# Dunni3/FlowMol

Hardware: AMD Instinct MI355X
Metric: molecules/sec at 250 timesteps (GEOM-drugs-sized graphs) (higher is better)
Workload: dtype f32

## Files before the change

flowmol_amd/csrc/fm_kernels.h:

```cpp
#pragma once
#include <type_traits>

#include "../../include/flowmol_hip.h"
#include "fm_device.h"

struct FmBatch {
    int B, N, E, U;
    int P;
    int n_tiles, tile_rows;
    const int* mol_node_off;
    const int* mol_edge_off;
    const int* mol_pair_off;
    int* node_mol;
    int* node_first_edge;
    int* e_src;
    int* e_dst;
    int* e_pair;
    int* p_e0;
    int* p_e1;
    int* pair_mol;
    const int* mol_tile_off;
    int4* tile_desc;
};

#define FM_CHUNK_E 16

static __global__ void __launch_bounds__(256) fm_k_batch_setup(FmBatch b) {
    const int gid = blockIdx.x * blockDim.x + threadIdx.x;
    if (gid < b.N) {
        int lo = 0, hi = b.B;
        while (hi - lo > 1) { const int mid = (lo + hi) >> 1; if (b.mol_node_off[mid] <= gid) lo = mid; else hi = mid; }
        b.node_mol[gid] = lo;
        const int n = b.mol_node_off[lo + 1] - b.mol_node_off[lo];
        b.node_first_edge[gid] = b.mol_edge_off[lo] + (gid - b.mol_node_off[lo]) * (n - 1);
    }
    if (gid < b.E) {
        int lo = 0, hi = b.B;
        while (hi - lo > 1) { const int mid = (lo + hi) >> 1; if (b.mol_edge_off[mid] <= gid) lo = mid; else hi = mid; }
        const int noff = b.mol_node_off[lo];
        const int n = b.mol_node_off[lo + 1] - noff;
        const int local = gid - b.mol_edge_off[lo];
        const int i = local / (n - 1), k = local % (n - 1);
        const int j = k + (k >= i ? 1 : 0);
        b.e_dst[gid] = noff + i;
        b.e_src[gid] = noff + j;
        const int a = i < j ? i : j, c = i < j ? j : i;
        const int pair = b.mol_pair_off[lo] + a * (2 * n - a - 1) / 2 + (c - a - 1);
        b.e_pair[gid] = pair;
        if (j < i) { b.p_e0[pair] = gid; b.pair_mol[pair] = lo; }
        else b.p_e1[pair] = gid;
    }
    if (gid < b.n_tiles) {
        int lo = 0, hi = b.B;
        while (hi - lo > 1) { const int mid = (lo + hi) >> 1; if (b.mol_tile_off[mid] <= gid) lo = mid; else hi = mid; }
        const int moff = b.mol_edge_off[lo];
        const int e0 = moff + (gid - b.mol_tile_off[lo]) * b.tile_rows;
        const int left = b.mol_edge_off[lo + 1] - e0;
        b.tile_desc[gid] = make_int4(e0, left < b.tile_rows ? left : b.tile_rows, moff, lo);
    }
}

enum FmMlpMode {
    FM_MLP_TABLE = 0,
    FM_MLP_SC_NODE = 1,
    FM_MLP_NODE_HEAD = 2,
    FM_MLP_EDGE_HEAD = 3,
    FM_MLP_SC_EDGE = 4,
    FM_MLP_NODE_LOSS = 5,
    FM_MLP_EDGE_LOSS = 6,
};
constexpr bool fm_mlp_node_head(int mode) { return mode == FM_MLP_NODE_HEAD || mode == FM_MLP_NODE_LOSS; }
constexpr bool fm_mlp_edge_head(int mode) { return mode == FM_MLP_EDGE_HEAD || mode == FM_MLP_EDGE_LOSS; }

__device__ __forceinline__ int fm_loss_target(const int* tok_t, const int* tok_1, int row, int mask) { return tok_t[row] == mask ? tok_1[row] : -1; }
template <bool LOSS>
__device__ __forceinline__ void fm_head_row(const float* lg, int n, float* out, int target) {
    if (LOSS && target < 0) { out[0] = 0.f; return; }
    float m = lg[0];
    for (int c = 1; c < n; ++c) m = fmaxf(m, lg[c]);
    float s = 0.f;
    for (int c = 0; c < n; ++c) s += expf(lg[c] - m);
    if (LOSS) out[0] = (logf(s) + m) - lg[target];
    else for (int c = 0; c < n; ++c) out[c] = expf(lg[c] - m) / s;
}

struct FmMlpArgs {
    int rows;
    int K1p;
    int H;
    int O;
    int ldx, ldh;
    const float2* W1; const float* b1;
    const float2* W2; const float* b2;
    const float* ln_g; const float* ln_b; int ln_n;
    const float* in;  int in_ld;
    int in_w;
    float* out; int out_ld;
    const float* s_tab; const int* tok_a; const int* tok_c; int n_c1;
    const float* prev_a; const float* prev_c; const float* prev_x; const float* x_t;
    int na, nc, ne;
    float rbf_mu_step, rbf_inv_sigma;
    float* out2;
    const float* ef; const int* p_e0; const int* p_e1;
    const int* e_src; const int* e_dst; const int* e_pair; const int* tok_e;
    const float* prev_e; const float* T1; const float* ef_tab;
    const float* emb_a; const float* emb_c; const float* temb; int ta, tc, tt;
    const float2* slabW0; float* slabQ0; const float2* slabW1; float* slabQ1;
    int tab_tiles; int tab_stride;
    const int* tab_slot; const int* node_mol; int slot_rows;
    const int* tgt_a; const int* tgt_c; const int* tgt_e;
};

template <int MODE, int TM>
__device__ __forceinline__ void fm_mlp2_tile(const FmMlpArgs& a, int tile, float* lds) {
    float* X = lds;
    float* Hb = lds + TM * a.ldx;
    int* meta = reinterpret_cast<int*>(Hb + TM * a.ldh);
    const int tid = threadIdx.x;
    const int row0 = tile * TM;

    if (MODE == FM_MLP_TABLE) {
        for (int idx = tid; idx < TM * a.K1p; idx += FM_THREADS) {
            const int r = idx / a.K1p, c = idx % a.K1p, row = row0 + r;
            float v = 0.f;
            if (row < a.rows) {
                if (a.in) v = (a.in_w == 0 || c < a.in_w) ? a.in[(size_t)row * a.in_ld + c] : 0.f;
                else {
                    const int ia = row / a.n_c1, ic = row % a.n_c1;
                    if (c < a.ta) v = a.emb_a ? a.emb_a[ia * a.ta + c] : (c == ia ? 1.f : 0.f);
                    else if (c < a.ta + a.tc) v = a.emb_c ? a.emb_c[ic * a.tc + (c - a.ta)] : ((c - a.ta) == ic ? 1.f : 0.f);
                    else if (c < a.ta + a.tc + a.tt) v = a.temb[c - a.ta - a.tc];
                }
            }
            X[r * a.ldx + c] = v;
        }
    } else if (MODE == FM_MLP_SC_NODE) {
        float* dd = reinterpret_cast<float*>(meta + TM);
        if (tid < TM) {
            const int n = row0 + tid;
            int tok = -1; float d = 0.f;
            if (n < a.rows) {
                tok = a.tok_a[n] * a.n_c1 + a.tok_c[n];
                if (a.tab_slot) tok += a.tab_slot[a.node_mol[n]] * a.slot_rows;
                d = fm_norm3(a.x_t[n * 3 + 0] - a.prev_x[n * 3 + 0], a.x_t[n * 3 + 1] - a.prev_x[n * 3 + 1], a.x_t[n * 3 + 2] - a.prev_x[n * 3 + 2]);
            }
            meta[tid] = tok; dd[tid] = d;
        }
        __syncthreads();
        {
            const auto rs = fm_buf(a.s_tab, 0x7fffffffu);
            constexpr int NQ = TM * 64 / FM_THREADS;
            float4 q[NQ];
#pragma unroll
            for (int k = 0; k < NQ; ++k) {
                const int idx = tid + k * FM_THREADS, r = idx >> 6, c4 = idx & 63;
                const int tok = meta[r];
                q[k] = fm_buf_f32x4(rs, tok >= 0 ? tok * 1024 + c4 * 16 : FM_BUF_OOB, 0);
            }
#pragma unroll
            for (int k = 0; k < NQ; ++k) {
                const int idx = tid + k * FM_THREADS, r = idx >> 6, c4 = idx & 63;
                *reinterpret_cast<float4*>(X + r * a.ldx + c4 * 4) = q[k];
            }
        }
        const int kin = a.na + a.nc + 32, kw = a.K1p - 256;
        for (int idx = tid; idx < TM * kw; idx += FM_THREADS) {
            const int r = idx / kw, c = idx % kw;
            const int n = row0 + r;
            float v = 0.f;
            if (meta[r] >= 0 && c < kin) {
                if (c < a.na) v = a.prev_a[(size_t)n * a.na + c];
                else if (c < a.na + a.nc) v = a.prev_c[(size_t)n * a.nc + (c - a.na)];
                else v = fm_rbf(dd[r], c - a.na - a.nc, a.rbf_mu_step, a.rbf_inv_sigma);
            }
            X[r * a.ldx + 256 + c] = v;
        }
    } else if (fm_mlp_node_head(MODE)) {
        const int left = a.rows - row0;
        const auto rs = fm_buf(a.in + (size_t)row0 * 256, (unsigned)(left < TM ? left : TM) * 1024u);
        constexpr int NQ = TM * 64 / FM_THREADS;
        float4 q[NQ];
#pragma unroll
        for (int k = 0; k < NQ; ++k) q[k] = fm_buf_f32x4(rs, (tid + k * FM_THREADS) * 16, 0);
#pragma unroll
        for (int k = 0; k < NQ; ++k) {
            const int idx = tid + k * FM_THREADS, r = idx >> 6, c4 = idx & 63;
            *reinterpret_cast<float4*>(X + r * a.ldx + c4 * 4) = q[k];
        }
    } else if (fm_mlp_edge_head(MODE)) {
        int* pr = meta + 3 * TM;
        if (tid < TM) {
            const int p = row0 + tid;
            meta[tid] = (p < a.rows) ? a.p_e0[p] : -1;
            pr[tid] = (p < a.rows) ? a.p_e1[p] : -1;
        }
        __syncthreads();
        constexpr int NQ = TM * 32 / FM_THREADS;
        float4 u0[NQ], u1[NQ];
#pragma unroll
        for (int k = 0; k < NQ; ++k) {
            const int idx = tid + k * FM_THREADS, r = idx >> 5, c4 = idx & 31;
            const int ea = meta[r], eb = pr[r];
            u0[k] = reinterpret_cast<const float4*>(a.ef)[(size_t)(ea < 0 ? 0 : ea) * 32 + c4];
            u1[k] = reinterpret_cast<const float4*>(a.ef)[(size_t)(eb < 0 ? 0 : eb) * 32 + c4];
        }
#pragma unroll
        for (int k = 0; k < NQ; ++k) {
            const int idx = tid + k * FM_THREADS, r = idx >> 5, c4 = idx & 31;
            const bool ok = meta[r] >= 0;
            float4 v;
            v.x = ok ? u0[k].x + u1[k].x : 0.f; v.y = ok ? u0[k].y + u1[k].y : 0.f;
            v.z = ok ? u0[k].z + u1[k].z : 0.f; v.w = ok ? u0[k].w + u1[k].w : 0.f;
            *reinterpret_cast<float4*>(X + r * a.ldx + 4 * c4) = v;
        }
    } else {
        float* dd = reinterpret_cast<float*>(meta + TM);
        int* pr = meta + 3 * TM;
        if (tid < TM) {
            const int p = row0 + tid;
            int tok = -1, ea = -1, eb = -1;
            float dt_ = 0.f, d1_ = 0.f;
            if (p < a.rows) {
                ea = a.p_e0[p]; eb = a.p_e1[p];
                const int i = a.e_src[ea], j = a.e_dst[ea];
                tok = a.tok_e[p];
                dt_ = fm_norm3(a.x_t[i * 3] - a.x_t[j * 3], a.x_t[i * 3 + 1] - a.x_t[j * 3 + 1], a.x_t[i * 3 + 2] - a.x_t[j * 3 + 2]) + 1e-8f;
                d1_ = fm_norm3(a.prev_x[i * 3] - a.prev_x[j * 3], a.prev_x[i * 3 + 1] - a.prev_x[j * 3 + 1],
                               a.prev_x[i * 3 + 2] - a.prev_x[j * 3 + 2]) + 1e-8f;
            }
            meta[tid] = tok; pr[tid] = eb; dd[2 * tid] = dt_; dd[2 * tid + 1] = d1_;
            meta[4 * TM + tid] = ea;
        }
        __syncthreads();
        for (int idx = tid; idx < TM * a.K1p; idx += FM_THREADS) {
            const int r = idx / a.K1p, c = idx % a.K1p;
            float v = 0.f;
            if (meta[r] >= 0) {
                if (c < a.ne) v = a.prev_e[(size_t)(row0 + r) * a.ne + c];
                else if (c < a.ne + 32)
                    v = fm_rbf(dd[2 * r + 1], c - a.ne, a.rbf_mu_step, a.rbf_inv_sigma) -
                        fm_rbf(dd[2 * r], c - a.ne, a.rbf_mu_step, a.rbf_inv_sigma);
            }
            X[r * a.ldx + c] = v;
        }
    }
    __syncthreads();

    fm_block_gemm<TM / 16, 1>(X, a.ldx, TM / 16, a.K1p / 8, a.W1, a.H / 16, [&](int row, int col, float v) {
        if (MODE == FM_MLP_SC_EDGE) { const int t = meta[row]; v += (t >= 0) ? a.T1[t * 128 + col] : 0.f; }
        else v += a.b1[col];
        Hb[row * a.ldh + col] = fm_silu(v);
    });
    __syncthreads();
    auto epi2 = [&](int row, int col, float v) {
        v += a.b2[col];
        if (MODE == FM_MLP_TABLE || MODE == FM_MLP_SC_NODE || MODE == FM_MLP_SC_EDGE) v = fm_silu(v);
        X[row * a.ldx + col] = v;
    };
    if (fm_mlp_node_head(MODE) || fm_mlp_edge_head(MODE)) fm_block_gemm<1, 1>(Hb, a.ldh, TM / 16, a.H / 8, a.W2, a.O / 16, epi2);
    else fm_block_gemm<TM / 16, 1>(Hb, a.ldh, TM / 16, a.H / 8, a.W2, a.O / 16, epi2);
    __syncthreads();

    constexpr int LPR = FM_THREADS / TM;
    const int r = tid / LPR, sub = tid % LPR;
    const int grow = row0 + r;
    if (MODE == FM_MLP_TABLE) {
        float mean, rstd;
        fm_row_stats<LPR>(X + r * a.ldx, a.ln_n, sub, mean, rstd);
        if (grow < a.rows) {
            float* o0 = a.out + (size_t)(a.p_e0 ? a.p_e0[grow] : grow) * a.out_ld;
            float* o1 = a.p_e1 ? a.out + (size_t)a.p_e1[grow] * a.out_ld : nullptr;
            for (int c = sub; c < a.O; c += LPR) {
                const float y = fm_fma((X[r * a.ldx + c] - mean) * rstd, a.ln_g[c], a.ln_b[c]);
                o0[c] = y;
                if (o1) o1[c] = y;
            }
        }
    } else if (MODE == FM_MLP_SC_NODE) {
        if (grow < a.rows) {
            const float* trow = a.s_tab + (size_t)meta[r] * 256;
            for (int c = sub * 4; c < 256; c += LPR * 4) {
                const float4 t = *reinterpret_cast<const float4*>(trow + c);
                const float4 x = *reinterpret_cast<const float4*>(X + r * a.ldx + c);
                *reinterpret_cast<float4*>(a.out + (size_t)grow * 256 + c) = make_float4(t.x + x.x, t.y + x.y, t.z + x.z, t.w + x.w);
            }
        }
    } else if (MODE == FM_MLP_SC_EDGE) {
        const bool slab = a.slabQ0 != nullptr;
        if (grow < a.rows) {
            const int ea = meta[4 * TM + r], eb = meta[3 * TM + r], tok = meta[r];
            for (int c = sub * 4; c < 128; c += LPR * 4) {
                const float4 t = *reinterpret_cast<const float4*>(a.ef_tab + tok * 128 + c);
                const float4 x = *reinterpret_cast<const float4*>(X + r * a.ldx + c);
                const float4 o = make_float4(t.x + x.x, t.y + x.y, t.z + x.z, t.w + x.w);
                *reinterpret_cast<float4*>(a.out + (size_t)ea * 128 + c) = o;
                *reinterpret_cast<float4*>(a.out + (size_t)eb * 128 + c) = o;
                if (slab) *reinterpret_cast<float4*>(Hb + r * a.ldh + 32 + c) = o;
            }
        }
        if (slab) {
            const float* dd = reinterpret_cast<const float*>(meta + TM);
            for (int idx = tid; idx < TM * 32; idx += FM_THREADS) {
                const int rr = idx >> 5, k = idx & 31;
                Hb[rr * a.ldh + k] = fm_rbf(dd[2 * rr], k, a.rbf_mu_step, a.rbf_inv_sigma);
            }
            __syncthreads();
            const int lane = tid & 63, wave = __builtin_amdgcn_readfirstlane(tid >> 6);
            const int left = a.rows - row0;
            auto slab_gemm = [&](const float2* __restrict__ W, float* Q) {
                constexpr int MT = TM / 16;
                f32x4 acc[MT][2];
#pragma unroll
                for (int i = 0; i < MT; ++i) { acc[i][0] = f32x4{0.f, 0.f, 0.f, 0.f}; acc[i][1] = f32x4{0.f, 0.f, 0.f, 0.f}; }
                fm_wave_gemm<MT, 2>(acc, Hb, 164, 20, W, 16, 2 * wave, lane);
                const auto rs = fm_buf(Q + (size_t)row0 * 256, (unsigned)(left < TM ? left : TM) * 1024u);
#pragma unroll
                for (int i = 0; i < MT; ++i)
#pragma unroll
                    for (int q = 0; q < 4; ++q)
                        fm_buf_store_f32x2(rs, (i * 16 + 4 * (lane >> 4) + q) * 1024 + (lane & 15) * 8, wave * 128, acc[i][0][q], acc[i][1][q]);
            };
            slab_gemm(a.slabW0, a.slabQ0);
            if (a.slabQ1) slab_gemm(a.slabW1, a.slabQ1);
        }
    } else {
        if (sub == 0 && grow < a.rows) {
            const float* lg = X + r * a.ldx;
            if (MODE == FM_MLP_NODE_HEAD) {
                fm_head_row<false>(lg, a.na, a.out + (size_t)grow * a.na, 0);
                fm_head_row<false>(lg + a.na, a.nc, a.out2 + (size_t)grow * a.nc, 0);
            } else if (MODE == FM_MLP_EDGE_HEAD) {
                fm_head_row<false>(lg, a.ne, a.out + (size_t)grow * a.ne, 0);
            } else if (MODE == FM_MLP_NODE_LOSS) {
                fm_head_row<true>(lg, a.na, a.out + grow, fm_loss_target(a.tok_a, a.tgt_a, grow, a.na));
                fm_head_row<true>(lg + a.na, a.nc, a.out2 + grow, fm_loss_target(a.tok_c, a.tgt_c, grow, a.nc));
            } else {
                fm_head_row<true>(lg, a.ne, a.out + grow, fm_loss_target(a.tok_e, a.tgt_e, grow, a.ne));
            }
        }
    }
}

template <int MODE, int TM = FM_TM>
__global__ void __launch_bounds__(FM_THREADS) fm_k_mlp2(FmMlpArgs a) {
    HIP_DYNAMIC_SHARED(float, lds)
    int tile = blockIdx.x;
    if (MODE == FM_MLP_TABLE && a.tab_tiles > 0) {
        const int tab = tile / a.tab_tiles;
        tile -= tab * a.tab_tiles;
        a.temb += tab * a.tt;
        a.out += (size_t)tab * a.tab_stride;
    }
    fm_mlp2_tile<MODE, TM>(a, tile, lds);
}

template <int MODE_A, int MODE_B, int TM = FM_TM>
__global__ void __launch_bounds__(FM_THREADS) fm_k_mlp2_pair(FmMlpArgs a, FmMlpArgs b, int tiles_a) {
    HIP_DYNAMIC_SHARED(float, lds)
    if ((int)blockIdx.x < tiles_a) fm_mlp2_tile<MODE_A, TM>(a, blockIdx.x, lds);
    else fm_mlp2_tile<MODE_B, TM>(b, (int)blockIdx.x - tiles_a, lds);
}

enum FmMlp4Mode { FM_MLP4_SC_NODE = 0, FM_MLP4_NODE_HEAD = 1, FM_MLP4_PROJ0 = 2, FM_MLP4_NODE_LOSS = 3 };
struct FmMlp4Args {
    int N;
    const void* W1q; const float* b1;
    const void* W2q; const float* b2;
    const float* s_tab; const int* tok_a; const int* tok_c; int n_c1;
    const int* tab_slot; const int* node_mol; int slot_rows;
    const float* prev_a; const float* prev_c; const float* prev_x; const float* x_t;
    int na, nc; float rbf_mu_step, rbf_inv_sigma;
    float* out; float* out2;
    const float* in;
    const void* Wps4; float* Ps; float* PV; int pv_w; float* v_init; int V; const float* x_src; float* x_dst;
    const int* tgt_a; const int* tgt_c;
};
#define FM_MLP4_LDX 324
#define FM_MLP4_LDH 260
#define FM_MLP4_LDS_BYTES ((4 * FM_MLP4_LDX + 4 * FM_MLP4_LDH + 16) * 4)

template <int MODE>
__device__ __forceinline__ void fm_mlp4_tile(const FmMlp4Args& a, int tile, float* lds) {
    constexpr int LDX = FM_MLP4_LDX, LDH = FM_MLP4_LDH;
    float* X = lds;
    float* Hb = X + 4 * LDX;
    int* meta = reinterpret_cast<int*>(Hb + 4 * LDH);
    float* dd = reinterpret_cast<float*>(meta + 4);
    const int tid = threadIdx.x, row0 = tile * 4;
    const int rows = a.N - row0 < 4 ? a.N - row0 : 4;
    if (MODE == FM_MLP4_SC_NODE) {
        if (tid < 4) {
            const int n = row0 + tid;
            int tok = -1; float d = 0.f;
            if (n < a.N) {
                tok = a.tok_a[n] * a.n_c1 + a.tok_c[n];
                if (a.tab_slot) tok += a.tab_slot[a.node_mol[n]] * a.slot_rows;
                d = fm_norm3(a.x_t[n * 3 + 0] - a.prev_x[n * 3 + 0], a.x_t[n * 3 + 1] - a.prev_x[n * 3 + 1], a.x_t[n * 3 + 2] - a.prev_x[n * 3 + 2]);
            }
            meta[tid] = tok; dd[tid] = d;
        }
        __syncthreads();
        if (tid < 256) {
            const int r = tid >> 6, c4 = tid & 63, tok = meta[r];
            *reinterpret_cast<float4*>(X + r * LDX + c4 * 4) = fm_buf_f32x4(fm_buf(a.s_tab), tok >= 0 ? tok * 1024 + c4 * 16 : FM_BUF_OOB, 0);
        } else {
            const int r = (tid - 256) >> 6, c = (tid - 256) & 63, n = row0 + r;
            float v = 0.f;
            if (meta[r] >= 0 && c < a.na + a.nc + 32) {
                if (c < a.na) v = a.prev_a[(size_t)n * a.na + c];
                else if (c < a.na + a.nc) v = a.prev_c[(size_t)n * a.nc + (c - a.na)];
                else v = fm_rbf(dd[r], c - a.na - a.nc, a.rbf_mu_step, a.rbf_inv_sigma);
            }
            X[r * LDX + 256 + c] = v;
        }
    } else {
        if (tid < 256)
            *reinterpret_cast<float4*>(X + (tid >> 6) * LDX + (tid & 63) * 4) = fm_buf_f32x4(fm_buf(a.in + (size_t)row0 * 256, (unsigned)rows * 1024u), tid * 16, 0);
        if (MODE == FM_MLP4_PROJ0) {
            for (int i = tid; i < rows * 3; i += FM_THREADS) a.x_dst[row0 * 3 + i] = a.x_src[row0 * 3 + i];
            for (int i = tid; i < rows * 3 * a.V; i += FM_THREADS) a.v_init[(size_t)row0 * 3 * a.V + i] = 0.f;
            for (int i = tid; i < rows * 3 * a.pv_w; i += FM_THREADS) a.PV[(size_t)row0 * 3 * a.pv_w + i] = 0.f;
        }
    }
    __syncthreads();
    if (MODE == FM_MLP4_PROJ0) {
        fm_rows4_linear<64, 4>(X, LDX, a.Wps4, [&](int r, int c, float v) { if (r < rows) a.Ps[(size_t)(row0 + r) * 256 + c] = v; });
        return;
    }
    if (MODE == FM_MLP4_SC_NODE)
        fm_rows4_linear<80, 4>(X, LDX, a.W1q, [&](int r, int c, float v) { Hb[r * LDH + c] = fm_silu(v + a.b1[c]); });
    else
        fm_rows4_linear<64, 4>(X, LDX, a.W1q, [&](int r, int c, float v) { Hb[r * LDH + c] = fm_silu(v + a.b1[c]); });
    if (MODE == FM_MLP4_SC_NODE) {
        fm_rows4_linear<64, 4>(Hb, LDH, a.W2q, [&](int r, int c, float v) {
            if (r < rows) a.out[(size_t)(row0 + r) * 256 + c] = a.s_tab[(size_t)meta[r] * 256 + c] + fm_silu(v + a.b2[c]);
        });
    } else {
        const int no = a.na + a.nc;
        fm_rows4_linear<64, 1>(Hb, LDH, a.W2q, [&](int r, int c, float v) { if (c < no) X[r * LDX + c] = v + a.b2[c]; });
        if (tid < rows) {
            const float* lg = X + tid * LDX;
            const int n = row0 + tid;
            if (MODE == FM_MLP4_NODE_LOSS) {
                fm_head_row<true>(lg, a.na, a.out + n, fm_loss_target(a.tok_a, a.tgt_a, n, a.na));
                fm_head_row<true>(lg + a.na, a.nc, a.out2 + n, fm_loss_target(a.tok_c, a.tgt_c, n, a.nc));
            } else {
                fm_head_row<false>(lg, a.na, a.out + (size_t)n * a.na, 0);
                fm_head_row<false>(lg + a.na, a.nc, a.out2 + (size_t)n * a.nc, 0);
            }
        }
    }
}

template <int MODE>
__global__ void __launch_bounds__(FM_THREADS) fm_k_mlp4(FmMlp4Args a) {
    HIP_DYNAMIC_SHARED(float, lds)
    fm_mlp4_tile<MODE>(a, blockIdx.x, lds);
}

template <int MODE4, int MODE_B>
__global__ void __launch_bounds__(FM_THREADS) fm_k_mlp4_pair(FmMlp4Args a, FmMlpArgs b, int tiles_a) {
    HIP_DYNAMIC_SHARED(float, lds)
    if ((int)blockIdx.x < tiles_a) fm_mlp4_tile<MODE4>(a, blockIdx.x, lds);
    else fm_mlp2_tile<MODE_B, 16>(b, (int)blockIdx.x - tiles_a, lds);
}

static __global__ void __launch_bounds__(256) fm_k_gather_rows(float* __restrict__ out, const float* __restrict__ tab, int width,
                                                         int rows, const int* __restrict__ tok_a, const int* __restrict__ tok_c,
                                                         int n_c1, const int* __restrict__ e_pair, const int* __restrict__ tab_slot,
                                                         const int* __restrict__ node_mol, int slot_rows) {
    const int w4 = width / 4;
    for (size_t idx = (size_t)blockIdx.x * blockDim.x + threadIdx.x; idx < (size_t)rows * w4; idx += (size_t)gridDim.x * blockDim.x) {
        const int row = (int)(idx / w4), c4 = (int)(idx % w4);
        int tok = e_pair ? tok_a[e_pair[row]] : tok_a[row] * n_c1 + tok_c[row];
        if (tab_slot) tok += tab_slot[node_mol[row]] * slot_rows;
        reinterpret_cast<float4*>(out)[idx] = reinterpret_cast<const float4*>(tab)[(size_t)tok * w4 + c4];
    }
}

struct FmProjArgs {
    int N;
    const float* s; const float* v;
    const float2* Wps; float* Ps;
    const float2* Wasd; float* Asd;
    const float2* Wpv; float* PV;
    int pv_w;
    float* v_init;
    const float* x_src; float* x_dst;
};

template <int V, int TM = FM_TM>
__global__ void __launch_bounds__(FM_THREADS) fm_k_node_proj(FmProjArgs a) {
    HIP_DYNAMIC_SHARED(float, lds)
    constexpr int LDS_ = 260;
    constexpr int LDV = V + 4;
    float* X = lds;
    float* Vt = lds + TM * LDS_;
    const int tid = threadIdx.x, row0 = blockIdx.x * TM;
    for (int idx = tid; idx < TM * 64; idx += FM_THREADS) {
        const int r = idx >> 6, c4 = idx & 63;
        float4 val = make_float4(0.f, 0.f, 0.f, 0.f);
        if (row0 + r < a.N) val = reinterpret_cast<const float4*>(a.s)[(size_t)(row0 + r) * 64 + c4];
        float* d = X + r * LDS_ + 4 * c4;
        *reinterpret_cast<float4*>(d) = val;
    }
    if (a.x_dst) {
        const int i0 = row0 * 3, i1 = (row0 + TM < a.N ? row0 + TM : a.N) * 3;
        for (int i = i0 + tid; i < i1; i += FM_THREADS) a.x_dst[i] = a.x_src[i];
    }
    if (a.PV) {
        const int rows = a.N - row0 < TM ? a.N - row0 : TM;
        const auto rs_v = fm_buf(a.v + (size_t)row0 * 3 * V, (unsigned)rows * (3 * V * 4));
        constexpr int V4 = V / 4, NCHK = TM * 3 * V4, NV = (NCHK + FM_THREADS - 1) / FM_THREADS;
        float4 qv[NV];
#pragma unroll
        for (int k = 0; k < NV; ++k) {
            const int idx = tid + k * FM_THREADS;
            if (a.v_init) {
                qv[k] = make_float4(0.f, 0.f, 0.f, 0.f);
                if (idx < rows * 3 * V4) reinterpret_cast<float4*>(a.v_init + (size_t)row0 * 3 * V)[idx] = qv[k];
            } else {
                qv[k] = fm_buf_f32x4(rs_v, idx < NCHK ? idx * 16 : FM_BUF_OOB, 0);
            }
        }
#pragma unroll
        for (int k = 0; k < NV; ++k) {
            const int idx = tid + k * FM_THREADS;
            if (idx < NCHK) {
                const int r = idx / (3 * V4), rem = idx % (3 * V4), c = rem / V4, u4 = rem % V4;
                *reinterpret_cast<float4*>(Vt + (c * TM + r) * LDV + u4 * 4) = qv[k];
            }
        }
    }
    __syncthreads();
    if (a.Ps)
        fm_block_gemm<TM / 16, 2>(X, LDS_, TM / 16, 32, a.Wps, 16, [&](int row, int col, float v) {
            if (row0 + row < a.N) a.Ps[(size_t)(row0 + row) * 256 + col] = v;
        });
    if (a.Asd)
        fm_block_gemm<TM / 16, 2>(X, LDS_, TM / 16, 32, a.Wasd, 16, [&](int row, int col, float v) {
            if (row0 + row < a.N) a.Asd[(size_t)(row0 + row) * 256 + col] = v;
        });
    if (a.PV)
        fm_block_gemm<1, 1>(Vt, LDV, 3 * TM / 16, V / 8, a.Wpv, a.pv_w / 16, [&](int row, int col, float v) {
            const int c = row / TM, r = row % TM;
            if (row0 + r < a.N) a.PV[((size_t)(row0 + r) * 3 + c) * a.pv_w + col] = v;
        });
}

struct FmDstProjArgs {
    int N;
    const float* s; const float* v;
    FmGvpW g;
    const float2* Wsd; float* Psd;
    const float2* Wpvd; float* PVd; int pv_w;
};

template <int V, int TM, int VD>
__global__ void __launch_bounds__(FM_THREADS) fm_k_dst_proj(FmDstProjArgs a) {
    typedef FmGvpTile<V, TM> T;
    HIP_DYNAMIC_SHARED(float, lds)
    float* X = lds;
    float* Vin = X + T::X_FLOATS;
    float* Vh = Vin + T::VIN_FLOATS;
    float* G = Vh + T::VH_FLOATS;
    const int tid = threadIdx.x, row0 = blockIdx.x * TM;
    {
        const int rows = a.N - row0 < TM ? a.N - row0 : TM;
        const auto rs_s = fm_buf(a.s + (size_t)row0 * 256, (unsigned)rows * 1024u);
        const auto rs_v = fm_buf(a.v + (size_t)row0 * 3 * V, (unsigned)rows * (3 * V * 4));
        constexpr int V4 = V / 4, NCHK = TM * 3 * V4;
        for (int idx = tid; idx < TM * 64; idx += FM_THREADS)
            *reinterpret_cast<float4*>(X + (idx >> 6) * FM_LDX + (idx & 63) * 4) = fm_buf_f32x4(rs_s, idx * 16, 0);
        for (int idx = tid; idx < NCHK; idx += FM_THREADS) {
            const int r = idx / (3 * V4), rem = idx % (3 * V4), c = rem / V4, u4 = rem % V4;
            *reinterpret_cast<float4*>(Vin + (c * TM + r) * T::LDVI + u4 * 4) = fm_buf_f32x4(rs_v, idx * 16, 0);
        }
    }
    __syncthreads();
    {
        FM_MARK_DECL
        float pre[TM / 16][2][4];
        fm_gvp_core<V, VD, false, true, TM, FM_THREADS>(X, Vin, Vh, G, a.g, pre FM_MARK_PASS(50));
    }
    constexpr int MT = TM / 16;
    fm_block_gemm<MT, 2>(X, FM_LDX, MT, 32, a.Wsd, 16, [&](int row, int col, float val) {
        if (row0 + row < a.N) a.Psd[(size_t)(row0 + row) * 256 + col] = val;
    });
    fm_block_gemm<1, 1>(Vin, T::LDVI, 3 * MT, 1, a.Wpvd, a.pv_w / 16, [&](int row, int col, float val) {
        const int c = row / TM, r = row % TM;
        if (row0 + r < a.N) a.PVd[((size_t)(row0 + r) * 3 + c) * a.pv_w + col] = val;
    });
}

struct FmMsgArgs {
    FmBatch b;
    const float* x;
    const float* ef;
    const float* Ps;
    const float* PV;
    const float* w0;
    const float* Psd;
    const float* PVd;
    FmGvpW g0, g1, g2;
    float* part_s;
    float* part_v;
    float rbf_mu_step, rbf_inv_sigma;
    float* dbg_s; float* dbg_v;
    const float* Q;
    int xcd_chunk;
};

template <int V, int TM, int NTH, int HX, int SP, int PQ = 0>
__global__ void __launch_bounds__(NTH) fm_k_edge_message(FmMsgArgs a) {
    static_assert(!(PQ && (SP || HX)), "the pair-slab instance exists for f32 models without destination features");
    typedef FmGvpTile<V, TM, HX> T;
    HIP_DYNAMIC_SHARED(float, lds)
    float* X = lds;
    constexpr int FMT = SP == 3 ? 1 : 0, NPL = SP == 2 ? 3 : 2;
    float* Vin = X + (SP ? TM * FM_LDP * NPL / 2 : T::X_FLOATS);
    float* Vh = Vin + T::VIN_FLOATS;
    float* G = SP ? Vh + TM * FM_LDG : Vh + T::VH_FLOATS;
    int* m_src = reinterpret_cast<int*>(SP ? Vh + T::VH_FLOATS : G + T::G_FLOATS);
    int* m_dst = m_src + TM;
    float* m_geo = reinterpret_cast<float*>(m_dst + TM);
    int* m_piece = reinterpret_cast<int*>(m_geo + 4 * TM);
    int* m_soff = m_piece + TM;
    int* m_doff = m_soff + TM;
    const int tid = threadIdx.x;
    const int tile = a.xcd_chunk > 0 ? (int)(blockIdx.x & 7) * a.xcd_chunk + (int)(blockIdx.x >> 3) : (int)blockIdx.x;
    if (tile >= a.b.n_tiles) return;
    const int4 td = a.b.tile_desc[tile];
    const int e0 = td.x, left = td.y, moff = td.z;
    FM_MARK_DECL
    constexpr int NEF = PQ ? 1 : TM * 32 / NTH;
    float4 efv[NEF];
    if constexpr (!PQ) {
        const auto rs = fm_buf(a.ef + (size_t)e0 * 128, (unsigned)left * 512u);
#pragma unroll
        for (int k = 0; k < NEF; ++k) efv[k] = (FM_ABLATE & 16) ? make_float4(0.1f, 0.2f, 0.3f, 0.4f) : fm_buf_f32x4(rs, tid * 16 + k * NTH * 16, 0);
    }
    if (PQ && tid < 64) {
        const int e = e0 + tid;
        const int pr = tid < left ? a.b.e_pair[e] : 0x7fffffff;
        int mn = pr;
#pragma unroll
        for (int o = 1; o < 64; o <<= 1) { const int t = __shfl_xor(mn, o); mn = t < mn ? t : mn; }
        if (tid < TM) m_doff[tid] = pr != 0x7fffffff ? (pr - mn) * 1024 : FM_BUF_OOB;
        if (tid == 0) m_doff[TM] = mn;
    }
    if (tid < TM) {
        const int e = e0 + tid;
        int s = -1, d = -1, piece = 0;
        float gx = 0.f, gy = 0.f, gz = 0.f, dist = 0.f;
        if (tid < left) {
            s = a.b.e_src[e]; d = a.b.e_dst[e];
            piece = (e - moff) / FM_CHUNK_E - (a.b.node_first_edge[d] - moff) / FM_CHUNK_E;
            const float dx = a.x[s * 3] - a.x[d * 3], dy = a.x[s * 3 + 1] - a.x[d * 3 + 1], dz = a.x[s * 3 + 2] - a.x[d * 3 + 2];
            dist = fm_norm3(dx, dy, dz) + 1e-8f;
            const float inv_d = __builtin_amdgcn_rcpf(dist);
            gx = dx * inv_d; gy = dy * inv_d; gz = dz * inv_d;
        }
        m_src[tid] = s; m_dst[tid] = d; m_piece[tid] = piece;
        m_soff[tid] = s >= 0 ? s * 1024 : FM_BUF_OOB;
        if (!PQ) m_doff[tid] = d >= 0 ? d * 1024 : FM_BUF_OOB;
        m_geo[4 * tid] = gx; m_geo[4 * tid + 1] = gy; m_geo[4 * tid + 2] = gz; m_geo[4 * tid + 3] = dist;
    }
    __syncthreads();
    FM_MARK(0);
    float pre[TM / 16][1024 / NTH][4];
    if (!(FM_ABLATE & 16)) fm_gather_pre<TM, NTH, false>(pre, a.Ps, a.b.N, m_soff);
    else { for (auto& p1 : pre) for (auto& p2 : p1) for (auto& p3 : p2) p3 = 0.25f; }
    if (HX > 0) fm_gather_pre<TM, NTH, true>(pre, a.Psd, a.b.N, m_doff);
    float preq[PQ ? TM / 16 : 1][PQ ? 1024 / NTH : 1][4];
    if constexpr (PQ) {
        static_assert(!PQ || NTH == 512, "Q rows are laid out for 8 waves x 2 column tiles");
        const int pmin = __builtin_amdgcn_readfirstlane(m_doff[TM]);
        const int lane = tid & 63, wave = __builtin_amdgcn_readfirstlane(tid >> 6);
        const auto rs = fm_buf(a.Q + (size_t)pmin * 256, 0x7ffffc00u);
#pragma unroll
        for (int i = 0; i < TM / 16; ++i)
#pragma unroll
            for (int r = 0; r < 4; ++r) {
                const float2 t = fm_buf_f32x2(rs, m_doff[i * 16 + 4 * (lane >> 4) + r] + (lane & 15) * 8, wave * 128);
                preq[i][0][r] = t.x; preq[i][1][r] = t.y;
            }
    }
    {
        constexpr int PVW = T::PVW, CB = PVW / 16, NCH = 3 * CB * TM, QN = NTH / 16, NP = (NCH + QN - 1) / QN;
        const int q = tid >> 4, j = tid & 15;
        const auto rs = fm_buf(a.PV, (unsigned)a.b.N * (unsigned)(3 * PVW * 4));
        const auto rsd = fm_buf(HX > 0 ? a.PVd : a.PV, (unsigned)a.b.N * (unsigned)(3 * PVW * 4));
        float pv[NP], w0v[NP];
#pragma unroll
        for (int p_ = 0; p_ < NP; ++p_) {
            const int ch = q + p_ * QN, r = ch % TM, ccb = ch / TM, c = ccb / CB, cb = ccb % CB;
            const int sidx = (NCH % QN == 0 || ch < NCH) ? m_src[r] : -1;
            pv[p_] = (FM_ABLATE & 16) ? 0.5f : fm_buf_f32(rs, sidx >= 0 ? sidx * (3 * PVW * 4) + j * 4 : FM_BUF_OOB, (c * PVW + cb * 16) * 4);
            if (HX > 0) {
                const int didx = (NCH % QN == 0 || ch < NCH) ? m_dst[r] : -1;
                pv[p_] += fm_buf_f32(rsd, didx >= 0 ? didx * (3 * PVW * 4) + j * 4 : FM_BUF_OOB, (c * PVW + cb * 16) * 4);
            }
            w0v[p_] = a.w0[cb * 16 + j];
        }
#pragma unroll
        for (int p_ = 0; p_ < NP; ++p_) {
            const int ch = q + p_ * QN, r = ch % TM, ccb = ch / TM, c = ccb / CB, cb = ccb % CB;
            if (NCH % QN == 0 || ch < NCH)
                Vh[(c * TM + r) * T::LDVH + cb * 16 + j] = fm_fma(m_geo[4 * r + c], w0v[p_], pv[p_]);
        }
    }
    if (SP) {
        unsigned short* XH = reinterpret_cast<unsigned short*>(X);
        unsigned short* XL = XH + TM * FM_LDP;
        constexpr int Z0 = 160 + T::KU0, Z1 = 256 + T::KU;
        for (int idx = tid; idx < TM * 24; idx += NTH) {
            const int r = idx / 24, c = idx % 24;
            if (Z0 + c < (Z0 + 31) / 32 * 32) { XH[r * FM_LDP + Z0 + c] = 0; XL[r * FM_LDP + Z0 + c] = 0; if (SP == 2) XL[TM * FM_LDP + r * FM_LDP + Z0 + c] = 0; }
            if (Z1 + c < 320) { XH[r * FM_LDP + Z1 + c] = 0; XL[r * FM_LDP + Z1 + c] = 0; if (SP == 2) XL[TM * FM_LDP + r * FM_LDP + Z1 + c] = 0; }
        }
        for (int idx = tid; idx < TM * 32; idx += NTH) {
            const int r = idx >> 5, k = idx & 31;
            if (SP == 2) fm_split3_store(XH, XL, r, k, fm_rbf(m_geo[4 * r + 3], k, a.rbf_mu_step, a.rbf_inv_sigma));
            else fm_split_store<FM_LDP, FMT>(XH, XL, r, k, fm_rbf(m_geo[4 * r + 3], k, a.rbf_mu_step, a.rbf_inv_sigma));
        }
#pragma unroll
        for (int k = 0; k < NEF; ++k) {
            const int idx = tid + k * NTH, r = idx >> 5, c4 = idx & 31;
            if (SP == 2) {
                fm_split3_store(XH, XL, r, 32 + 4 * c4 + 0, efv[k].x); fm_split3_store(XH, XL, r, 32 + 4 * c4 + 1, efv[k].y);
                fm_split3_store(XH, XL, r, 32 + 4 * c4 + 2, efv[k].z); fm_split3_store(XH, XL, r, 32 + 4 * c4 + 3, efv[k].w);
            } else {
                fm_split_store<FM_LDP, FMT>(XH, XL, r, 32 + 4 * c4 + 0, efv[k].x); fm_split_store<FM_LDP, FMT>(XH, XL, r, 32 + 4 * c4 + 1, efv[k].y);
                fm_split_store<FM_LDP, FMT>(XH, XL, r, 32 + 4 * c4 + 2, efv[k].z); fm_split_store<FM_LDP, FMT>(XH, XL, r, 32 + 4 * c4 + 3, efv[k].w);
            }
        }
    } else if constexpr (!PQ) {
    for (int idx = tid; idx < TM * 32; idx += NTH) {
        const int r = idx >> 5, k = idx & 31;
        X[r * FM_LDX + k] = fm_rbf(m_geo[4 * r + 3], k, a.rbf_mu_step, a.rbf_inv_sigma);
    }
#pragma unroll
    for (int k = 0; k < NEF; ++k) {
        const int idx = tid + k * NTH, r = idx >> 5, c4 = idx & 31;
        *reinterpret_cast<float4*>(X + r * FM_LDX + 32 + 4 * c4) = efv[k];
    }
    }
    if constexpr (PQ) {
#pragma unroll
        for (int i = 0; i < TM / 16; ++i)
#pragma unroll
            for (int j = 0; j < 1024 / NTH; ++j)
#pragma unroll
                for (int r = 0; r < 4; ++r) pre[i][j][r] += preq[i][j][r];
    }
    __syncthreads();
    FM_MARK(1);
    constexpr bool PF = V == 32 && TM == 32 && NTH == 512 && SP == 0 && HX == 0;
    float2 bw[V / 8][2];
    fm_gvp_core_pf<V, V, true, true, TM, NTH, HX, SP, false, PQ != 0, 0, PF>(X, Vin, Vh, G, a.g0, a.g1, bw, pre FM_MARK_PASS(10));
    fm_gvp_core_pf<V, V, false, true, TM, NTH, HX, SP, false, false, 0, PF>(X, Vin, Vh, G, a.g1, a.g2, bw, pre FM_MARK_PASS(20));
    fm_gvp_core_pf<V, V, false, true, TM, NTH, HX, SP, true, false, 0, PF>(X, Vin, Vh, G, a.g2, a.g2, bw, pre FM_MARK_PASS(30));

    if (a.dbg_s) {
        for (int idx = tid; idx < TM * 256; idx += NTH) {
            const int r = idx >> 8, c = idx & 255;
            if (m_src[r] >= 0) a.dbg_s[(size_t)(e0 + r) * 256 + c] = X[r * FM_LDX + c];
        }
        for (int idx = tid; idx < 3 * TM * V; idx += NTH) {
            const int row = idx / V, u = idx % V, c = row / TM, r = row % TM;
            if (m_src[r] >= 0) a.dbg_v[((size_t)(e0 + r) * 3 + c) * V + u] = Vin[row * T::LDVI + u];
        }
    }
    FM_MARK(40);
    static_assert(NTH >= 512 && 3 * V <= 128 && TM <= 64, "waves 0..3 own the 256 scalar columns, waves 4..5 the 3*V vector columns (the others idle here; 1024-thread instances were measured in round 6: profiles/r06d_*)");
    if (!(FM_ABLATE & 8)) {
        const int wave = __builtin_amdgcn_readfirstlane(tid >> 6), lane = tid & 63;
        const int lr = lane < TM ? lane : TM - 1;
        const int myd = m_dst[lr];
        const int nxd = m_dst[lr + 1 < TM ? lr + 1 : TM - 1];
        const unsigned long long ends = __ballot(lane < TM && myd >= 0 && (lr + 1 == TM || nxd != myd || (lr & (FM_CHUNK_E - 1)) == FM_CHUNK_E - 1));
        const bool is_s = wave < 4;
        const int cv = tid - 256;
        auto column_sums = [&](const float* vp, auto stride_c, float* out_base, unsigned row_bytes, int col) {
            constexpr int STRIDE = decltype(stride_c)::value;
            float val[TM];
#pragma unroll
            for (int r = 0; r < TM; ++r) val[r] = vp[r * STRIDE];
            float run = 0.f;
#pragma unroll
            for (int r = 0; r < TM; ++r) {
                run += val[r];
                if ((ends >> r) & 1ull) {
                    const int d = __builtin_amdgcn_readfirstlane(m_dst[r]), pcr = __builtin_amdgcn_readfirstlane(m_piece[r]);
                    const size_t slot = (size_t)d * a.b.P + pcr;
                    fm_buf_store_f32(fm_buf(reinterpret_cast<const char*>(out_base) + slot * row_bytes, row_bytes), col * 4, 0, run);
                    run = 0.f;
                }
            }
        };
        if (is_s) column_sums(X + tid, std::integral_constant<int, FM_LDX>{}, a.part_s, 1024u, tid);
        else if (cv < 3 * V) column_sums(Vin + (cv / V) * TM * T::LDVI + (cv % V), std::integral_constant<int, T::LDVI>{}, a.part_v, 3 * V * 4u, cv);
    }
    FM_MARK(41);
}

struct FmNodeUpdArgs {
    FmBatch b;
    float* s; float* v;
    const float* part_s; const float* part_v;
    float inv_z;
    FmGvpW g0, g1, g2;
    const float* ln1_g; const float* ln1_b; const float* ln2_g; const float* ln2_b;
    float* agg_s; float* agg_v;
    const float2* Wps; float* Ps;
    const float2* Wpv; float* PV;
    const float2* Wasd; float* Asd;
    FmGvpW p0, p1, p2; float* x;
    const void* Wps_sp; const void* Wasd_sp;
    const void* Wps4; const void* Wasd4;
    int s_real;
};

template <int V, int TM, int SP = 0>
__device__ __forceinline__ void fm_gvp_layernorm_tile(float* X, float* Vin, const float* g, const float* b_,
                                                      int row0, int nrows, float* out_s, float* out_v, int s_width = 256, int rows_valid = TM) {
    typedef FmGvpTile<V, TM> T;
    constexpr int LPR = FM_THREADS / TM;
    const int tid = threadIdx.x, r = tid / LPR, sub = tid % LPR;
    float mean, rstd;
    fm_row_stats<LPR>(X + r * FM_LDX, s_width, sub, mean, rstd);
    float q = 0.f;
    for (int u = fm_ln_sub<LPR>(sub); u < V; u += FmLnLanes<LPR>::value) {
        const float vx = Vin[(0 * TM + r) * T::LDVI + u], vy = Vin[(1 * TM + r) * T::LDVI + u], vz = Vin[(2 * TM + r) * T::LDVI + u];
        q += fmaxf(fm_fma(vz, vz, fm_fma(vy, vy, vx * vx)), 1e-8f);
    }
    q = fm_group_sum<FmLnLanes<LPR>::value>(q);
    const float vn = __builtin_amdgcn_sqrtf(fm_fma(q, 1.0f / (float)V, 1e-5f)) + 1e-5f;
    const float inv_vn = __builtin_amdgcn_rcpf(vn);
    const bool valid = r < rows_valid && row0 + r < nrows;
    if constexpr (SP) {
        float ys[256 / LPR];
#pragma unroll
        for (int k = 0; k < 256 / LPR; ++k) {
            const int c = sub + k * LPR;
            ys[k] = fm_fma((X[r * FM_LDX + c] - mean) * rstd, g[c], b_[c]);
            if (out_s && valid) out_s[(size_t)(row0 + r) * 256 + c] = ys[k];
        }
        __syncthreads();
        unsigned short* XH = reinterpret_cast<unsigned short*>(X);
        unsigned short* XL = XH + TM * FM_LDP;
#pragma unroll
        for (int k = 0; k < 256 / LPR; ++k) fm_split_store<FM_LDP, (SP == 3 ? 1 : 0)>(XH, XL, r, sub + k * LPR, ys[k]);
        for (int c = 256 + V + 8 + sub; c < 320; c += LPR) { XH[r * FM_LDP + c] = 0; XL[r * FM_LDP + c] = 0; }
    } else {
    for (int c = sub; c < 256; c += LPR) {
        const float y = fm_fma((X[r * FM_LDX + c] - mean) * rstd, g[c], b_[c]);
        X[r * FM_LDX + c] = y;
        if (out_s && valid) out_s[(size_t)(row0 + r) * 256 + c] = y;
    }
    }
    for (int u = sub; u < V; u += LPR)
#pragma unroll
        for (int c = 0; c < 3; ++c) {
            const float y = Vin[(c * TM + r) * T::LDVI + u] * inv_vn;
            Vin[(c * TM + r) * T::LDVI + u] = y;
            if (out_v && valid) out_v[((size_t)(row0 + r) * 3 + c) * V + u] = y;
        }
    __syncthreads();
}

template <int V, int TM, bool NARROW, int SP, int RG = 0>
__global__ void __launch_bounds__(FM_THREADS) fm_k_node_update(FmNodeUpdArgs a) {
    static_assert(RG == 0 || (4 * RG <= TM && !NARROW && !SP), "the 4 RG-node instances exist for f32 full-width models");
    typedef FmGvpTile<V, TM> T;
    constexpr int RV = RG ? 4 * RG : TM;
    HIP_DYNAMIC_SHARED(float, lds)
    float* X = lds;
    float* Vin = X + (SP ? TM * FM_LDP : T::X_FLOATS);
    float* Vh = Vin + T::VIN_FLOATS;
    float* G = SP ? Vh + TM * FM_LDG : Vh + T::VH_FLOATS;
    const int tid = threadIdx.x, row0 = blockIdx.x * RV;
    const int N = a.b.N, P = a.b.P;
    const int rows = N - row0 < RV ? N - row0 : RV;
    int* r_np = reinterpret_cast<int*>(G);
    float* r_iz = G + TM;
    if (tid < TM) {
        const int n = row0 + tid;
        int np = 0;
        float iz = a.inv_z;
        if (n < N && tid < RV) {
            const int m = a.b.node_mol[n];
            const int deg = a.b.mol_node_off[m + 1] - a.b.mol_node_off[m] - 1;
            if (deg > 0) {
                const int fe = a.b.node_first_edge[n] - a.b.mol_edge_off[m];
                np = (fe + deg - 1) / FM_CHUNK_E - fe / FM_CHUNK_E + 1;
            }
            if (iz < 0.f) iz = deg > 0 ? 1.0f / (float)deg : 0.f;
        }
        r_np[tid] = np; r_iz[tid] = iz;
    }
    __syncthreads();
    const auto rs_s = fm_buf(a.s + (size_t)row0 * 256, (unsigned)rows * 1024u);
    const auto rs_v = fm_buf(a.v + (size_t)row0 * 3 * V, (unsigned)rows * (3 * V * 4));
    {
        const auto rs_p = fm_buf(a.part_s + (size_t)row0 * P * 256, (unsigned)rows * (unsigned)P * 1024u);
        constexpr int NQ = TM * 64 / FM_THREADS;
#pragma unroll
        for (int k = 0; k < NQ; ++k) {
            const int idx = tid + k * FM_THREADS, r = idx >> 6, c4 = idx & 63;
            const int np = r_np[r];
            const float4 sv = fm_buf_f32x4(rs_s, (r * 256 + c4 * 4) * 4, 0);
            float4 acc = make_float4(0.f, 0.f, 0.f, 0.f);
            for (int p0 = 0; p0 < P; p0 += 4) {
                float4 q[4];
#pragma unroll
                for (int j = 0; j < 4; ++j) q[j] = fm_buf_f32x4(rs_p, p0 + j < np ? ((r * P + p0 + j) * 256 + c4 * 4) * 4 : FM_BUF_OOB, 0);
#pragma unroll
                for (int j = 0; j < 4; ++j) { acc.x += q[j].x; acc.y += q[j].y; acc.z += q[j].z; acc.w += q[j].w; }
            }
            const float iz = r_iz[r];
            acc.x *= iz; acc.y *= iz; acc.z *= iz; acc.w *= iz;
            if (a.agg_s && r < rows) *reinterpret_cast<float4*>(a.agg_s + (size_t)(row0 + r) * 256 + c4 * 4) = acc;
            *reinterpret_cast<float4*>(X + r * FM_LDX + c4 * 4) = make_float4(sv.x + acc.x, sv.y + acc.y, sv.z + acc.z, sv.w + acc.w);
        }
    }
    {
        const auto rs_p = fm_buf(a.part_v + (size_t)row0 * P * 3 * V, (unsigned)rows * (unsigned)P * (3 * V * 4));
        constexpr int V4 = V / 4, NCHK = TM * 3 * V4;
        for (int idx = tid; idx < NCHK; idx += FM_THREADS) {
            const int r = idx / (3 * V4), rem = idx % (3 * V4), c = rem / V4, u4 = rem % V4;
            const int np = r_np[r];
            const float4 vv = fm_buf_f32x4(rs_v, ((r * 3 + c) * V + u4 * 4) * 4, 0);
            float4 acc = make_float4(0.f, 0.f, 0.f, 0.f);
            for (int p0 = 0; p0 < P; p0 += 4) {
                float4 q[4];
#pragma unroll
                for (int j = 0; j < 4; ++j) q[j] = fm_buf_f32x4(rs_p, p0 + j < np ? (((r * P + p0 + j) * 3 + c) * V + u4 * 4) * 4 : FM_BUF_OOB, 0);
#pragma unroll
                for (int j = 0; j < 4; ++j) { acc.x += q[j].x; acc.y += q[j].y; acc.z += q[j].z; acc.w += q[j].w; }
            }
            const float iz = r_iz[r];
            acc.x *= iz; acc.y *= iz; acc.z *= iz; acc.w *= iz;
            if (a.agg_v && r < rows) *reinterpret_cast<float4*>(a.agg_v + ((size_t)(row0 + r) * 3 + c) * V + u4 * 4) = acc;
            *reinterpret_cast<float4*>(Vin + (c * TM + r) * T::LDVI + u4 * 4) = make_float4(vv.x + acc.x, vv.y + acc.y, vv.z + acc.z, vv.w + acc.w);
        }
    }
    __syncthreads();
    const int s_width = NARROW ? a.s_real : 256;
    constexpr bool PF = V == 32 && TM == 32 && SP == 0 && RG == 0 && !NARROW;
    float2 bw[V / 8][2];
    if constexpr (PF) {
        const int lane = tid & 63, wave = __builtin_amdgcn_readfirstlane(tid >> 6);
        if (wave & 1) fm_wfrag_request<V / 8, 2, 1>(bw, a.g0.Wv1 + 2 * 64, (size_t)3 * 64, lane);
        else fm_wfrag_request<V / 8, 2, 2>(bw, a.g0.Wv1, (size_t)3 * 64, lane);
    }
    fm_gvp_layernorm_tile<V, TM, SP>(X, Vin, a.ln1_g, a.ln1_b, row0, N, a.s, a.v, s_width, RV);
    {
        FM_MARK_DECL
        float pre[TM / 16][2][4];
        fm_gvp_core_pf<V, V, false, true, TM, FM_THREADS, 0, SP, false, false, RG, PF>(X, Vin, Vh, G, a.g0, a.g1, bw, pre FM_MARK_PASS(50));
        fm_gvp_core_pf<V, V, false, true, TM, FM_THREADS, 0, SP, false, false, RG, PF>(X, Vin, Vh, G, a.g1, a.g2, bw, pre FM_MARK_PASS(50));
        fm_gvp_core_pf<V, V, false, true, TM, FM_THREADS, 0, SP, true, false, RG, PF>(X, Vin, Vh, G, a.g2, a.g2, bw, pre FM_MARK_PASS(50));
    }
    {
        constexpr int NQ = TM * 64 / FM_THREADS;
        float4 sv[NQ];
#pragma unroll
        for (int k = 0; k < NQ; ++k) { const int idx = tid + k * FM_THREADS; sv[k] = fm_buf_f32x4(rs_s, ((idx >> 6) * 256 + (idx & 63) * 4) * 4, 0); }
#pragma unroll
        for (int k = 0; k < NQ; ++k) {
            const int idx = tid + k * FM_THREADS;
            float4* xp = reinterpret_cast<float4*>(X + (idx >> 6) * FM_LDX + (idx & 63) * 4);
            float4 x = *xp;
            x.x += sv[k].x; x.y += sv[k].y; x.z += sv[k].z; x.w += sv[k].w;
            *xp = x;
        }
        constexpr int V4 = V / 4, NCHK = TM * 3 * V4;
        for (int idx = tid; idx < NCHK; idx += FM_THREADS) {
            const int r = idx / (3 * V4), rem = idx % (3 * V4), c = rem / V4, u4 = rem % V4;
            const float4 vv = fm_buf_f32x4(rs_v, ((r * 3 + c) * V + u4 * 4) * 4, 0);
            float4* vp = reinterpret_cast<float4*>(Vin + (c * TM + r) * T::LDVI + u4 * 4);
            float4 x = *vp;
            x.x += vv.x; x.y += vv.y; x.z += vv.z; x.w += vv.w;
            *vp = x;
        }
    }
    __syncthreads();
    fm_gvp_layernorm_tile<V, TM, SP>(X, Vin, a.ln2_g, a.ln2_b, row0, N, a.s, a.v, s_width, RV);
    constexpr int MT = TM / 16;
    if constexpr (SP) {
        const int lane = tid & 63, wave = __builtin_amdgcn_readfirstlane(tid >> 6);
        const unsigned short* XH = reinterpret_cast<const unsigned short*>(X);
        const unsigned short* XL = XH + TM * FM_LDP;
        auto project = [&](const void* wsp, float* out) {
            f32x4 acc[MT][2];
#pragma unroll
            for (int i = 0; i < MT; ++i)
#pragma unroll
                for (int j = 0; j < 2; ++j) acc[i][j] = f32x4{0.f, 0.f, 0.f, 0.f};
            fm_wave_gemm_sp<MT, 2, FM_LDP, (SP == 3 ? 1 : 0)>(acc, XH, XL, 0, 8, wsp, 16, 2 * wave, lane);
#pragma unroll
            for (int i = 0; i < MT; ++i)
#pragma unroll
                for (int j = 0; j < 2; ++j)
#pragma unroll
                    for (int r = 0; r < 4; ++r) {
                        const int row = i * 16 + 4 * (lane >> 4) + r;
                        if (row0 + row < N) out[(size_t)(row0 + row) * 256 + (2 * wave + j) * 16 + (lane & 15)] = acc[i][j][r] * (1.0f / fm_sp_wscale<(SP == 3 ? 1 : 0)>());
                    }
        };
        if (a.Ps) project(a.Wps_sp, a.Ps);
        if (a.Asd) project(a.Wasd_sp, a.Asd);
    } else if constexpr (RG > 0) {
        const int lane = tid & 63, wave = __builtin_amdgcn_readfirstlane(tid >> 6);
        const void* wq = wave < 4 ? a.Wps4 : a.Wasd4;
        float* out = wave < 4 ? a.Ps : a.Asd;
        if (out) {
            f32x4 acc[RG];
#pragma unroll
            for (int rg = 0; rg < RG; ++rg) acc[rg] = f32x4{0.f, 0.f, 0.f, 0.f};
            if (!(FM_ABLATE & 32)) fm_wave_gemm4<64, RG>(acc, X, FM_LDX, wq, wave & 3, lane);
#pragma unroll
            for (int rg = 0; rg < RG; ++rg)
#pragma unroll
                for (int r = 0; r < 4; ++r)
                    if (4 * rg + r < rows) out[(size_t)(row0 + 4 * rg + r) * 256 + 64 * (wave & 3) + lane] = acc[rg][r];
        }
    } else {
    if (a.Ps)
        fm_block_gemm<MT, 2>(X, FM_LDX, MT, 32, a.Wps, 16, [&](int row, int col, float val) {
            if (row0 + row < N) a.Ps[(size_t)(row0 + row) * 256 + col] = val;
        });
    if (a.Asd)
        fm_block_gemm<MT, 2>(X, FM_LDX, MT, 32, a.Wasd, 16, [&](int row, int col, float val) {
            if (row0 + row < N) a.Asd[(size_t)(row0 + row) * 256 + col] = val;
        });
    }
    if (a.PV)
        fm_block_gemm<1, 1>(Vin, T::LDVI, 3 * MT, V / 8, a.Wpv, (V + 16) / 16, [&](int row, int col, float val) {
// ... 1104 lines not shown
```

Baseline: 63.37.

## Derive edge endpoints from packed tile descriptors instead of gathering index arrays

Packs node offset, node count and first destination row into the tile descriptor. For small f32 tiles the message kernel now recomputes src, dst, piece and pair indices arithmetically per lane instead of loading e_src/e_dst/e_pair/node_first_edge. It also spreads the per-row coordinate and PV loads across all 16-lane groups so they issue before the first barrier, removing the serial single-thread-per-row prologue. Risks include bit-packing limits on node offsets and counts, and the float-reciprocal division correction for index decoding.

```diff
diff --git a/flowmol_amd/csrc/fm_kernels.h b/flowmol_amd/csrc/fm_kernels.h
--- a/flowmol_amd/csrc/fm_kernels.h
+++ b/flowmol_amd/csrc/fm_kernels.h
@@ -3,6 +3,7 @@
 
 #include "../../include/flowmol_hip.h"
 #include "fm_device.h"
+#include "fm_tile_desc.h"
 
 struct FmBatch {
     int B, N, E, U;
@@ -56,7 +57,10 @@
         const int moff = b.mol_edge_off[lo];
         const int e0 = moff + (gid - b.mol_tile_off[lo]) * b.tile_rows;
         const int left = b.mol_edge_off[lo + 1] - e0;
-        b.tile_desc[gid] = make_int4(e0, left < b.tile_rows ? left : b.tile_rows, moff, lo);
+        const int noff = b.mol_node_off[lo], n = b.mol_node_off[lo + 1] - noff;
+        int4 d;
+        fm_tile_encode(FmTile{e0, left < b.tile_rows ? left : b.tile_rows, moff, n, noff, (e0 - moff) / (n - 1)}, d.x, d.y, d.z, d.w);
+        b.tile_desc[gid] = d;
     }
 }
 
@@ -630,8 +634,10 @@
     const int tid = threadIdx.x;
     const int tile = a.xcd_chunk > 0 ? (int)(blockIdx.x & 7) * a.xcd_chunk + (int)(blockIdx.x >> 3) : (int)blockIdx.x;
     if (tile >= a.b.n_tiles) return;
-    const int4 td = a.b.tile_desc[tile];
-    const int e0 = td.x, left = td.y, moff = td.z;
+    const int4 tdp = a.b.tile_desc[tile];
+    const FmTile td = fm_tile_decode(tdp.x, tdp.y, tdp.z, tdp.w);
+    [[maybe_unused]] const int e0 = td.e0, left = td.left, moff = td.moff;
+    constexpr bool ENTRY = SP == 0 && TM <= 32 && NTH == 512;
     FM_MARK_DECL
     constexpr int NEF = PQ ? 1 : TM * 32 / NTH;
     float4 efv[NEF];
@@ -640,16 +646,51 @@
 #pragma unroll
         for (int k = 0; k < NEF; ++k) efv[k] = (FM_ABLATE & 16) ? make_float4(0.1f, 0.2f, 0.3f, 0.4f) : fm_buf_f32x4(rs, tid * 16 + k * NTH * 16, 0);
     }
+    constexpr int QN = NTH / 16;
+    const int q = tid >> 4, j = tid & 15;
+    [[maybe_unused]] const int er_row = q % TM;
+    [[maybe_unused]] const int er_half = ENTRY && QN > TM ? __builtin_amdgcn_readfirstlane(q / TM) : 0;
+    [[maybe_unused]] const float er_inv = __builtin_amdgcn_rcpf((float)(td.n - 1));
+    [[maybe_unused]] const bool er_live = er_row < left;
+    [[maybe_unused]] FmTileRow er{-1, -1, 0, 0};
+    if constexpr (ENTRY) er = fm_tile_row(td, er_inv, er_row);
     if (PQ && tid < 64) {
-        const int e = e0 + tid;
-        const int pr = tid < left ? a.b.e_pair[e] : 0x7fffffff;
+        [[maybe_unused]] const int e = e0 + tid;
+        int pr = 0x7fffffff;
+        if constexpr (ENTRY) { const int t = fm_tile_row(td, er_inv, tid).pair; pr = tid < left ? t : pr; }
+        else if (tid < left) pr = a.b.e_pair[e];
         int mn = pr;
 #pragma unroll
         for (int o = 1; o < 64; o <<= 1) { const int t = __shfl_xor(mn, o); mn = t < mn ? t : mn; }
         if (tid < TM) m_doff[tid] = pr != 0x7fffffff ? (pr - mn) * 1024 : FM_BUF_OOB;
         if (tid == 0) m_doff[TM] = mn;
     }
-    if (tid < TM) {
+    typedef FmGvpTile<V, TM, HX> TT;
+    constexpr int PVW_ = TT::PVW, CB_ = PVW_ / 16, NCH_ = 3 * CB_ * TM, NP_ = ENTRY ? (NCH_ + QN - 1) / QN : 1;
+    [[maybe_unused]] float e_pv[NP_], e_w0[NP_], e_xs[3], e_xd[3];
+    if constexpr (ENTRY) {
+        static_assert(QN % TM == 0, "every 16-lane group fills one row");
+        const auto rx = fm_buf(a.x, (unsigned)a.b.N * 12u);
+        const int xs = er_live ? er.src * 12 : FM_BUF_OOB, xd = er_live ? er.dst * 12 : FM_BUF_OOB;
+#pragma unroll
+        for (int c = 0; c < 3; ++c) { e_xs[c] = fm_buf_f32(rx, xs, c * 4); e_xd[c] = fm_buf_f32(rx, xd, c * 4); }
+        const auto rs = fm_buf(a.PV, (unsigned)a.b.N * (unsigned)(3 * PVW_ * 4));
+        const auto rsd = fm_buf(HX > 0 ? a.PVd : a.PV, (unsigned)a.b.N * (unsigned)(3 * PVW_ * 4));
+        const int svo = er_live ? er.src * (3 * PVW_ * 4) + j * 4 : FM_BUF_OOB, dvo = er_live ? er.dst * (3 * PVW_ * 4) + j * 4 : FM_BUF_OOB;
+#pragma unroll
+        for (int p_ = 0; p_ < NP_; ++p_) {
+            const int ccb = er_half + p_ * (QN / TM), c = ccb / CB_, cb = ccb % CB_;
+            const bool in = NCH_ % QN == 0 || ccb < 3 * CB_;
+            e_pv[p_] = (FM_ABLATE & 16) ? 0.5f : fm_buf_f32(rs, in ? svo : FM_BUF_OOB, (c * PVW_ + cb * 16) * 4);
+            if (HX > 0) e_pv[p_] += fm_buf_f32(rsd, in ? dvo : FM_BUF_OOB, (c * PVW_ + cb * 16) * 4);
+            e_w0[p_] = a.w0[cb * 16 + j];
+        }
+        if (j == 0 && q < TM) {
+            m_src[q] = er_live ? er.src : -1; m_dst[q] = er_live ? er.dst : -1; m_piece[q] = er_live ? er.piece : 0;
+            m_soff[q] = er_live ? er.src * 1024 : FM_BUF_OOB;
+            if (!PQ) m_doff[q] = er_live ? er.dst * 1024 : FM_BUF_OOB;
+        }
+    } else if (tid < TM) {
         const int e = e0 + tid;
         int s = -1, d = -1, piece = 0;
         float gx = 0.f, gy = 0.f, gz = 0.f, dist = 0.f;
@@ -686,9 +727,21 @@
                 preq[i][0][r] = t.x; preq[i][1][r] = t.y;
             }
     }
-    {
-        constexpr int PVW = T::PVW, CB = PVW / 16, NCH = 3 * CB * TM, QN = NTH / 16, NP = (NCH + QN - 1) / QN;
-        const int q = tid >> 4, j = tid & 15;
+    [[maybe_unused]] float e_dist = 0.f;
+    if constexpr (ENTRY) {
+        const float dx = e_xs[0] - e_xd[0], dy = e_xs[1] - e_xd[1], dz = e_xs[2] - e_xd[2];
+        const float dist = fm_norm3(dx, dy, dz) + 1e-8f;
+        const float inv_d = __builtin_amdgcn_rcpf(dist);
+        const float g[3] = {dx * inv_d, dy * inv_d, dz * inv_d};
+        e_dist = er_live ? dist : 0.f;
+#pragma unroll
+        for (int p_ = 0; p_ < NP_; ++p_) {
+            const int ccb = er_half + p_ * (QN / TM), c = ccb / CB_, cb = ccb % CB_;
+            if (NCH_ % QN == 0 || ccb < 3 * CB_)
+                Vh[(c * TM + er_row) * T::LDVH + cb * 16 + j] = fm_fma(c == 0 ? g[0] : c == 1 ? g[1] : g[2], e_w0[p_], e_pv[p_]);
+        }
+    } else {
+        constexpr int PVW = T::PVW, CB = PVW / 16, NCH = 3 * CB * TM, NP = (NCH + QN - 1) / QN;
         const auto rs = fm_buf(a.PV, (unsigned)a.b.N * (unsigned)(3 * PVW * 4));
         const auto rsd = fm_buf(HX > 0 ? a.PVd : a.PV, (unsigned)a.b.N * (unsigned)(3 * PVW * 4));
         float pv[NP], w0v[NP];
@@ -736,6 +789,13 @@
             }
         }
     } else if constexpr (!PQ) {
+    if constexpr (ENTRY) {
+#pragma unroll
+        for (int k0 = 0; k0 < 32; k0 += 16 * (QN / TM)) {
+            const int k = k0 + 16 * er_half + j;
+            X[er_row * FM_LDX + k] = fm_rbf(e_dist, k, a.rbf_mu_step, a.rbf_inv_sigma);
+        }
+    } else
     for (int idx = tid; idx < TM * 32; idx += NTH) {
         const int r = idx >> 5, k = idx & 31;
         X[r * FM_LDX + k] = fm_rbf(m_geo[4 * r + 3], k, a.rbf_mu_step, a.rbf_inv_sigma);
diff --git a/flowmol_amd/csrc/fm_tile_desc.h b/flowmol_amd/csrc/fm_tile_desc.h
--- /dev/null
+++ b/flowmol_amd/csrc/fm_tile_desc.h
@@ -0,0 +1,55 @@
+#pragma once
+
+#if defined(__HIPCC__)
+#define FM_HD __host__ __device__ __forceinline__
+#else
+#define FM_HD inline
+#endif
+
+#ifndef FM_CHUNK_E
+#define FM_CHUNK_E 16
+#endif
+
+struct FmTile {
+    int e0;
+    int left;
+    int moff;
+    int n;
+    int node_off;
+    int i0;
+};
+
+struct FmTileRow {
+    int src, dst;
+    int piece;
+    int pair;
+};
+
+FM_HD void fm_tile_encode(const FmTile& t, int& x, int& y, int& z, int& w) {
+    x = t.e0; y = t.moff; z = t.node_off | (t.left << 21); w = t.n | (t.i0 << 15);
+}
+
+FM_HD FmTile fm_tile_decode(int x, int y, int z, int w) {
+    FmTile t;
+    t.e0 = x; t.moff = y; t.node_off = z & 0x1fffff; t.left = (int)((unsigned)z >> 21); t.n = w & 0x7fff; t.i0 = (int)((unsigned)w >> 15);
+    return t;
+}
+
+FM_HD FmTileRow fm_tile_row(const FmTile& t, float inv, int row) {
+    const int m = t.n - 1;
+    const int local = t.e0 - t.moff + row;
+    const int q = local - t.i0 * m;
+    int di = (int)((float)q * inv);
+    int k = q - di * m;
+    if (k < 0) { --di; k += m; }
+    if (k >= m) { ++di; k -= m; }
+    const int i = t.i0 + di, j = k + (k >= i ? 1 : 0);
+    const int a = i < j ? i : j, c = i < j ? j : i;
+    FmTileRow r;
+    r.dst = t.node_off + i;
+    r.src = t.node_off + j;
+    static_assert(FM_CHUNK_E == 16, "chunk quotients are shifts");
+    r.piece = (local >> 4) - ((local - k) >> 4);
+    r.pair = (t.moff >> 1) + ((a * (2 * t.n - a - 1)) >> 1) + (c - a - 1);
+    return r;
+}
```

After: 64.05, median of 6. 1.01x the previous value.
